# qlchan/cronsun

Hardware: AMD Instinct MI355X
Metric: fire events materialised/sec (1M rules × 24h) + HBM GB/s at 1/2/4/8 GPU (higher is better)
Workload: dtype int64

## Files before the change

### cronsun_amd/csrc/cg_api_internal.h

```cpp
#pragma once
#include <hip/hip_runtime.h>

#include <algorithm>
#include <mutex>
#include <string>
#include <vector>

#include "../../include/cronsun_gpu.h"
#include "cg_kernels.h"
#include "cg_zone.h"

int cg_fail(int code, const std::string& msg);
int cg_hip_check(hipError_t e, const char* what);

#define HIPCHK(x)                    \
  do {                               \
    int _rc = cg_hip_check((x), #x); \
    if (_rc != CG_OK) return _rc;    \
  } while (0)

struct alignas(16) RuleInfo {
  int32_t cnt, off, first, st;
};

struct alignas(16) PairRec {
  int32_t rule, dst, x, st;
};

inline int gridn(int64_t n, int threads, int cap) {
  int64_t b = (n + threads - 1) / threads;
  if (b < 1) b = 1;
  return int(std::min<int64_t>(b, cap));
}

template <class T>
struct DBuf {
  T* p = nullptr;
  size_t cap = 0;
  int ensure(size_t n) {
    if (n <= cap) return CG_OK;
    if (p) (void)hipFree(p);
    p = nullptr;
    size_t want = std::max(n, cap + cap / 4);
    hipError_t e = hipMalloc(&p, want * sizeof(T));
    if (e != hipSuccess) {
      e = hipMalloc(&p, n * sizeof(T));
      if (e != hipSuccess) {
        p = nullptr;
        cap = 0;
        return cg_hip_check(e, "hipMalloc");
      }
      want = n;
    }
    cap = want;
    return CG_OK;
  }
  void release() {
    if (p) (void)hipFree(p);
    p = nullptr;
    cap = 0;
  }
};

struct RulesStore {
  DBuf<int64_t> nid_off, gid_off, ex_off, group_off;
  DBuf<int32_t> nids, gids, ex, group_nodes, rule_job;
  DBuf<int32_t> next_same, prev_same;
  bool has_dup = false;
  DBuf<uint8_t> group_exists, job_pause;
  int32_t n_nodes = 0, n_groups = 0, n_rules = 0, n_jobs = 0;
  uint64_t serial = 0;
  void release() {
    nid_off.release(); gid_off.release(); ex_off.release(); group_off.release();
    nids.release(); gids.release(); ex.release(); group_nodes.release(); rule_job.release();
    next_same.release(); prev_same.release();
    group_exists.release(); job_pause.release();
  }
};

struct RunSet {
  DBuf<int64_t> run_anchor, run_off, offsets, block_run;
  DBuf<int32_t> run_count;
  DBuf<uint32_t> run_dmask;
  DBuf<char> scan_tmp, plan_dev;
  DBuf<unsigned long long> stuck;
  int64_t* res_host = nullptr;
  int64_t* res_dev = nullptr;
  char* plan_pin = nullptr;
  size_t plan_pin_cap = 0;
  cg::Plan plan;
  cg::PlanArgs pa{};
  bool plan_valid = false;
  uint64_t plan_zone = 0;
  int64_t plan_t0 = 0, plan_t1 = 0;
  bool plan_lock_table = false;
  bool armed = false;
  int64_t R = 0, cap = 0;
  bool has_walk() const { return (plan.flags & (cg::kPlanT0Walk | cg::kPlanWalkSegs)) != 0; }
  int ensure_res() {
    if (res_host) return CG_OK;
    HIPCHK(hipHostMalloc(reinterpret_cast<void**>(&res_host), 16, hipHostMallocMapped | hipHostMallocCoherent));
    HIPCHK(hipHostGetDevicePointer(reinterpret_cast<void**>(&res_dev), res_host, 0));
    res_host[0] = 0;
    res_host[1] = -1;
    return CG_OK;
  }
  void release() {
    run_anchor.release(); run_off.release(); offsets.release(); block_run.release();
    run_count.release(); run_dmask.release(); scan_tmp.release(); plan_dev.release(); stuck.release();
    if (res_host) (void)hipHostFree(res_host);
    if (plan_pin) (void)hipHostFree(plan_pin);
    res_host = res_dev = nullptr;
    plan_pin = nullptr;
    plan_pin_cap = 0;
  }
};

struct AsyncSet {
  RunSet rs;
  hipEvent_t written = nullptr;
  hipEvent_t done = nullptr;
  int tslot = 0;
  int tprev = -1;
  bool pending = false;
  void release() {
    rs.release();
    if (written) (void)hipEventDestroy(written), written = nullptr;
    done = nullptr;
  }
};

struct PnWindow {
  DBuf<RuleInfo> rule_info;
  DBuf<int64_t> seg_cnt, seg_pos;
  DBuf<int32_t> seg_nrec;
  DBuf<PairRec> recs;
  DBuf<uint32_t> tickets;
  int64_t* node_off = nullptr;
  void* scan_tmp = nullptr;
  int64_t* res_host = nullptr;
  int64_t* res_dev = nullptr;
  const int64_t* offsets = nullptr;
  const int64_t* times = nullptr;
  int64_t t0 = 0;
  int32_t N = 0, K = 0, B = 0;
  int ensure_res() {
    if (res_host) return CG_OK;
    HIPCHK(hipHostMalloc(reinterpret_cast<void**>(&res_host), 32, hipHostMallocMapped | hipHostMallocCoherent));
    HIPCHK(hipHostGetDevicePointer(reinterpret_cast<void**>(&res_dev), res_host, 0));
    res_host[0] = res_host[1] = res_host[2] = 0;
    return CG_OK;
  }
  void release() {
    rule_info.release(); seg_cnt.release(); seg_pos.release(); seg_nrec.release();
    recs.release(); tickets.release();
    if (res_host) (void)hipHostFree(res_host);
    res_host = res_dev = nullptr;
  }
};

struct PnAsyncSet {
  RunSet rm;
  PnWindow w;
  DBuf<int64_t> times, node_off;
  DBuf<char> seg_tmp;
  hipEvent_t side_done = nullptr, written = nullptr, nw0 = nullptr, nw1 = nullptr;
  bool pending = false;
  bool timed = false;
  int64_t t0 = 0, t1 = 0, node_cap = 0, rm_cap = 0;
  int32_t N = 0;
  void release() {
    rm.release();
    w.release();
    times.release(); node_off.release(); seg_tmp.release();
    for (hipEvent_t* e : {&side_done, &written, &nw0, &nw1})
      if (*e) (void)hipEventDestroy(*e), *e = nullptr;
  }
};

struct cg_ctx {
  int device = 0;
  int write_blocks = 1024;
  int write_blocks_ov = 1024;
  hipStream_t st = nullptr;
  hipEvent_t ev[8] = {};
  hipEvent_t pev[4] = {};
  std::mutex mu;
  float kt[23] = {0, 0, 0, 0, 0, 0, 0, 0, 0, 0, 0, 0, 0, 0, 0, 0, 0, 0, 0, 0, 0, 0, 0};
  int phase_timing = 2;

  std::vector<char> plan_host;
  DBuf<char> plan_dev;

  RunSet rs;
  DBuf<int64_t> times, nb_in, nb_out, lt_avg;
  DBuf<int32_t> lt_kind;
  DBuf<char> scan_tmp;
  DBuf<unsigned long long> cksum;
  int64_t last_E = 0, last_R = 0;

#ifndef CG_ASYNC_SETS
#define CG_ASYNC_SETS 3
#endif
  static constexpr int kAsyncSets = CG_ASYNC_SETS;
  AsyncSet as[kAsyncSets];
  int as_next = 0, as_last = -1;
  hipStream_t st_cs = nullptr;
  hipEvent_t cs_done[kAsyncSets] = {};
  int async_rc = 0;
  std::string async_msg;
  double wr_ms_sum = 0;
  int wr_n = 0;
  hipStream_t st_w1 = nullptr;
  DBuf<int64_t> times2;
  bool ov_on = true;
  bool ov_active = false;
  bool w1_dirty = false;
  unsigned wr_call = 0;
  int times_last = 0;
  static constexpr int kTimeRing = kAsyncSets + 1;
  hipEvent_t tw0[kTimeRing] = {}, tw1[kTimeRing] = {};
  int tw_next = 0, tw_prev = -1;
  int64_t* result_times() const { return times_last ? times2.p : times.p; }

  static constexpr int kPnSets = 3;
  PnAsyncSet pns[kPnSets];
  int pa_next = 0, pa_last = -1;
  int pa_rc = 0;
  std::string pa_msg;
  double nw_ms_sum = 0;
  int nw_n = 0;
  int64_t pa_en_sum = 0;

  DBuf<int64_t> rn_off, node_off, node_time, nt_off, rs_off, seg_pair;
  DBuf<int32_t> rn_cnt, rn_nodes, pair_node, pair_rule, node_rule, nt_rule, rs_hist;
  PnWindow pn;
  DBuf<int32_t> ts_cnt, ts_tile_node, ts_hist, node_rule2;
  DBuf<int64_t> ts_base, ts_off, node_time2, ts_node_off;
  DBuf<int64_t> ts_start;
  DBuf<int32_t> ts_hi;
  int64_t pn_t0 = 0, pn_t1 = 0;
  RulesStore rules;
  int64_t pn_E = 0, pn_nnz = 0, pn_N = 0;
  bool pn_valid = false;
  int64_t pn_R = INT64_MAX;
  DBuf<int64_t> mr_rb, mr_tp, mr_t;
  DBuf<int32_t> mr_r;
  uint64_t pn_cache_serial = 0;
  int pn_cache_mode = -1;
  int node_order = CG_NODE_ORDER_RULE;
  bool pn_time_ordered = false;
  int32_t pn_B = 0, pn_K = 0;
  hipStream_t st_ot = nullptr;
  hipEvent_t ot_fork = nullptr, ot_join = nullptr;

  DBuf<int32_t> pf_rules, pf_chunk_cnt;
  DBuf<int64_t> pf_totals, pf_nodes, pf_part, pf_chunk_off;
  int64_t pf_R = 0;
  int32_t pf_N = 0, pf_B = 0;
  bool pf_valid = false, pf_has_nodes = false;
  int pf_kind = CG_PROFILE_STARTS;
  DBuf<int64_t> pf_dur, pf_peak;
  DBuf<int32_t> pf_peak_bucket;
  bool pf_peaks_valid = false;
  DBuf<char> pf_admit_units;
  DBuf<uint8_t> pf_admit_flag;
  DBuf<unsigned long long> pf_lock_stuck;
  hipEvent_t pfev[9] = {};
  uint64_t nt_gen = 0, pf_nt_gen = 0;
  int64_t pf_nnz = 0;
  DBuf<int32_t> tr_rule, tr_cnt, tr_nlisted, tr_ncontrib, tr_bucket, tr_part_nz;
  DBuf<unsigned long long> tr_part;
  int32_t tr_rows = 0, tr_k = 0;
  bool tr_valid = false;
  float tr_ms[3] = {0, 0, 0};
  hipEvent_t trev[3] = {};

  void free_all() {
    tr_rule.release(); tr_cnt.release(); tr_nlisted.release(); tr_ncontrib.release();
    tr_bucket.release(); tr_part_nz.release(); tr_part.release();
    for (hipEvent_t& e : trev)
      if (e) (void)hipEventDestroy(e), e = nullptr;
    for (AsyncSet& a : as) a.release();
    for (PnAsyncSet& a : pns) a.release();
    for (hipEvent_t& e : cs_done)
      if (e) (void)hipEventDestroy(e), e = nullptr;
    for (hipEvent_t* ring : {tw0, tw1})
      for (int i = 0; i < kTimeRing; i++)
        if (ring[i]) (void)hipEventDestroy(ring[i]), ring[i] = nullptr;
    if (st_cs) (void)hipStreamDestroy(st_cs);
    st_cs = nullptr;
    if (st_w1) (void)hipStreamDestroy(st_w1);
    st_w1 = nullptr;
    times2.release();
    if (ot_fork) (void)hipEventDestroy(ot_fork), ot_fork = nullptr;
    if (ot_join) (void)hipEventDestroy(ot_join), ot_join = nullptr;
    if (st_ot) (void)hipStreamDestroy(st_ot);
    st_ot = nullptr;
    plan_dev.release();
    rs.release(); times.release();
    nb_in.release(); nb_out.release(); lt_avg.release(); lt_kind.release();
    scan_tmp.release(); cksum.release();
    rn_off.release(); node_off.release(); node_time.release(); nt_off.release(); rs_off.release();
    seg_pair.release(); rn_cnt.release(); rn_nodes.release();
    pair_node.release(); pair_rule.release(); node_rule.release(); nt_rule.release();
    rs_hist.release(); pn.release(); rules.release();
    ts_cnt.release(); ts_tile_node.release(); ts_hist.release(); node_rule2.release();
    ts_start.release(); ts_hi.release();
    ts_base.release(); ts_off.release(); node_time2.release(); ts_node_off.release();
    mr_rb.release(); mr_tp.release(); mr_t.release(); mr_r.release();
    pf_rules.release(); pf_chunk_cnt.release(); pf_totals.release(); pf_nodes.release();
    pf_part.release(); pf_chunk_off.release();
    pf_dur.release(); pf_peak.release(); pf_peak_bucket.release();
    pf_admit_units.release(); pf_admit_flag.release(); pf_lock_stuck.release();
    for (hipEvent_t& e : pfev)
      if (e) (void)hipEventDestroy(e), e = nullptr;
  }
};

struct cg_rules {
  cg_ctx* ctx = nullptr;
  RulesStore st;
};

struct cg_zone {
  cg::ZoneRules rules;
  uint64_t serial;
};

struct cg_specs {
  cg_ctx* ctx = nullptr;
  cg::DSpec* d = nullptr;
  size_t n = 0;
  bool owner = false;
};

int pack_spec(const cg_schedule& s, cg::DSpec* d);
int upload_plan(cg_ctx* c, const cg::Plan& plan, int64_t t0, int64_t t1, cg::PlanArgs* pa);
struct PlanLayout {
  size_t o_when, o_off, o_seg, o_dt, bytes;
};
PlanLayout plan_layout(const cg::Plan& plan);
void plan_pack(const cg::Plan& plan, const PlanLayout& L, char* dst);
int plan_args(const cg::Plan& plan, const PlanLayout& L, char* dev_base, int64_t t0, int64_t t1,
              cg::PlanArgs* pa);
int run_set_count_scan(RunSet& rs, const cg_specs* s, const cg_zone* z, int64_t t0, int64_t t1, int64_t map_cap,
                       hipStream_t st, hipEvent_t* ev, bool* empty, bool lock_table = false);
int sync_count_scan(cg_ctx* c, const cg_specs* s, const cg_zone* z, int64_t t0, int64_t t1, bool* empty,
                    int64_t map_cap = 0, bool lock_table = false);
void run_set_write_enqueue(const RunSet& rs, const cg_specs* s, int64_t cap, int64_t* out, int blocks,
                           hipStream_t st, hipEvent_t after_cf = nullptr);
std::string stuck_msg(unsigned long long rule);
int expand_device_locked(cg_ctx* c, const cg_specs* s, const cg_zone* z, int64_t t0, int64_t t1,
                         int64_t* n_events);
int async_drain(cg_ctx* c);
int ensure_async(cg_ctx* c);
bool async_pending(const cg_ctx* c);
int pn_async_drain(cg_ctx* c);
bool pn_async_pending(const cg_ctx* c);
int upload_rules(const cg_rules_in* in, RulesStore* st, hipStream_t s);
int rule_nodes_locked(cg_ctx* c, const RulesStore& st, int mode, int64_t* nnz_out);
int transpose_locked(cg_ctx* c, int64_t nnz, int32_t N);
constexpr int kNodeChunk = 512;
int profile_node_peaks_enqueue(cg_ctx* c);
int64_t radix_hist_words(int64_t n);
void radix_by_key_enqueue(hipStream_t st, uint32_t* k0, int32_t* v0, uint32_t* k1, int32_t* v1, int64_t n,
                          int32_t N, int32_t* hist, int64_t* off, void* scan_tmp, bool* in_second);
void launch_node_bounds(hipStream_t st, const uint32_t* keys, int64_t n, int32_t N, int64_t* off);
constexpr int kInTimes = 0, kIn16 = 1, kInPacked = 2;
bool pn_pack_ok(int64_t R);
struct TileCut {
  const int64_t* seg_pos = nullptr;
  int32_t K = 1, B = 1;
  int64_t R = 0;
};
int order_merge_enqueue(cg_ctx* c, const int64_t* node_off, int32_t N, int64_t cap, int64_t t0, int64_t H,
                        hipStream_t st, int in_mode, int64_t* err, const TileCut& cut = TileCut());
constexpr const char* kOrderCheckMsg =
    "time-order pass: a sorted chunk came out of (time, rule) order (its LDS-atomic ranks were not in lane order)";
int order_by_time_locked(cg_ctx* c, int in_mode = 0);
int launch_node_place(cg_ctx* c, hipStream_t st, int32_t N, const int64_t* src_off, int64_t src_shift,
                      const int64_t* src_time, const int32_t* src_rule, int32_t rule_add, const int64_t* dst_start,
                      int64_t* dst_time, int32_t* dst_rule);
int launch_span_place(cg_ctx* c, hipStream_t st, int64_t n, const int64_t* src_time, const int32_t* src_rule,
                      int32_t rule_add, int64_t* dst_time, int32_t* dst_rule);
int launch_node_counts(cg_ctx* c, hipStream_t st, int64_t* d_counts);
int merge_ranks_locked(cg_ctx* c, hipStream_t st, int32_t N, int32_t W, const int64_t* h_rb, int64_t* d_time,
                       int32_t* d_rule, int64_t scratch_ev, DBuf<int64_t>& scr_t, DBuf<int32_t>& scr_r);
constexpr int kMergeMaxRanks = 64;
bool order_lsd_only();
```

### cronsun_amd/csrc/cg_pernode.hip

```cpp
#include <hip/hip_runtime.h>

#include <algorithm>
#include <atomic>
#include <cstdlib>
#include <cstring>
#include <unordered_map>
#include <vector>

#include "../../include/cronsun_gpu.h"
#include "cg_api_internal.h"
#include "cg_kernels.h"

using namespace cg;

namespace {


__global__ void k_seg_bounds(const int64_t* __restrict__ nt_off, const int32_t* __restrict__ nt_rule,
                             int32_t N, int32_t K, int32_t B, int64_t* __restrict__ seg_pair) {
  const int64_t t = blockIdx.x * int64_t(blockDim.x) + threadIdx.x;
  const int64_t NK = int64_t(N) * K;
  if (t > NK) return;
  if (t == NK) {
    seg_pair[t] = nt_off[N];
    return;
  }
  const int32_t n = int32_t(t / K), k = int32_t(t - int64_t(n) * K);
  int64_t lo = nt_off[n], hi = nt_off[n + 1];
  const int64_t x = int64_t(k) * B;
  while (lo < hi) {
    const int64_t mid = (lo + hi) >> 1;
    if (int64_t(nt_rule[mid]) < x) lo = mid + 1;
    else hi = mid;
  }
  seg_pair[t] = lo;
}

#ifndef CG_NODE_AP
#define CG_NODE_AP 1
#endif
constexpr int kApRules = 256;
inline int64_t rule_info_slots(int64_t R) { return std::max<int64_t>(R, 1); }
__global__ __launch_bounds__(256) void k_rule_info(const int64_t* __restrict__ rule_off,
                                                    const int64_t* __restrict__ times, int64_t R, int64_t t0,
                                                    int32_t B, int64_t cap, RuleInfo* __restrict__ info,
                                                    int64_t* __restrict__ err) {
  __shared__ int64_t off[kApRules + 1];
  __shared__ int64_t step[kApRules];
  __shared__ int32_t ok[kApRules];
  const int64_t r0 = int64_t(blockIdx.x) * kApRules;
  const int nr = int(R - r0 < kApRules ? R - r0 : kApRules);
  const int tid = threadIdx.x;
  if (rule_off[R] > cap) {
    if (tid < nr) info[r0 + tid] = RuleInfo{0, 0, 0, 0};
    return;
  }
  const int64_t band_lo = rule_off[(r0 / B) * B];
  if (r0 % B == 0 && threadIdx.x == 0 && rule_off[r0 + B < R ? r0 + B : R] - band_lo > (int64_t(1) << 30))
    err[0] = 1;
  int64_t first = 0, cnt = 0;
  if (tid < nr) {
    const int64_t a = rule_off[r0 + tid];
    cnt = rule_off[r0 + tid + 1] - a;
    first = cnt > 0 ? times[a] : 0;
    off[tid] = a;
    step[tid] = cnt > 1 ? times[a + 1] - first : 1;
    ok[tid] = CG_NODE_AP;
  }
  if (tid == 0) off[nr] = rule_off[r0 + nr];
  __syncthreads();
  const int64_t e_end = off[nr];
  constexpr int kRiUnroll = 4;
  for (int64_t e0 = off[0] + tid; e0 + 1 < e_end; e0 += int64_t(blockDim.x) * kRiUnroll) {
    int64_t ta[kRiUnroll], tb[kRiUnroll];
#pragma unroll
    for (int u = 0; u < kRiUnroll; u++) {
      const int64_t e = e0 + int64_t(u) * blockDim.x;
      const int64_t ec = e + 1 < e_end ? e : e_end - 2;
      ta[u] = times[ec];
      tb[u] = times[ec + 1];
    }
#pragma unroll
    for (int u = 0; u < kRiUnroll; u++) {
      const int64_t e = e0 + int64_t(u) * blockDim.x;
      if (e + 1 >= e_end) break;
      int lo = 0, hi = nr - 1;
      while (lo < hi) {
        const int mid = (lo + hi + 1) >> 1;
        if (off[mid] <= e) lo = mid;
        else hi = mid - 1;
      }
      if (e + 1 < off[lo + 1] && tb[u] - ta[u] != step[lo]) ok[lo] = 0;
    }
  }
  __syncthreads();
  if (tid < nr) {
    const int64_t rel = first - t0, s = step[tid];
    const bool prog = cnt > 0 && ok[tid] && rel >= 0 && rel <= INT32_MAX && s > 0 && s <= INT32_MAX;
    info[r0 + tid] = RuleInfo{int32_t(cnt), int32_t(off[tid] - band_lo),
                              prog ? int32_t(rel) : 0, prog ? int32_t(s) : 0};
  }
}

__device__ __forceinline__ int32_t scan_halves(int32_t x) {
  x += __builtin_amdgcn_update_dpp(0, x, 0x111, 0xf, 0xf, true);
  x += __builtin_amdgcn_update_dpp(0, x, 0x112, 0xf, 0xf, true);
  x += __builtin_amdgcn_update_dpp(0, x, 0x114, 0xf, 0xf, true);
  x += __builtin_amdgcn_update_dpp(0, x, 0x118, 0xf, 0xf, true);
  x += __builtin_amdgcn_update_dpp(0, x, 0x142, 0xa, 0xf, false);
  return x;
}
__device__ __forceinline__ int32_t half_total(int32_t incl) {
  const int32_t lo = __builtin_amdgcn_readlane(incl, 31), hi = __builtin_amdgcn_readlane(incl, 63);
  return (threadIdx.x & 63) < 32 ? lo : hi;
}

#ifndef CG_SEG_PAIRS_PER_LANE
#define CG_SEG_PAIRS_PER_LANE 8
#endif
constexpr int kSegPairsPerLane = CG_SEG_PAIRS_PER_LANE;
constexpr int kSegWavesPerSimd = 1;

__global__ __launch_bounds__(256, kSegWavesPerSimd) void k_seg_records(const int64_t* __restrict__ seg_pair,
                                                      const int32_t* __restrict__ nt_rule,
                                                      const int64_t* __restrict__ rule_off,
                                                      const RuleInfo* __restrict__ info, int32_t N,
                                                      int32_t K, int32_t B, int64_t R,
                                                      int64_t* __restrict__ seg_cnt,
                                                      int32_t* __restrict__ seg_nrec,
                                                      PairRec* __restrict__ recs,
                                                      uint32_t* __restrict__ tickets,
                                                      int64_t* __restrict__ err, int32_t xg) {
  if (blockIdx.x == 0)
    for (int i = threadIdx.x; i < kTicketGroups * kTicketStride; i += blockDim.x) tickets[i] = 0;
  const int32_t grp = int32_t(blockIdx.x % unsigned(xg));
  const int64_t nb_g = (int64_t(gridDim.x) - grp + xg - 1) / xg;
  const int64_t lb = blockIdx.x / unsigned(xg);
  const int64_t nbands = (int64_t(K) - grp + xg - 1) / xg;
  const int64_t NKg = nbands * N;
  constexpr int L = 32;
  constexpr int P = kSegPairsPerLane;
  const int lane = threadIdx.x & 63, hl = lane & (L - 1);
  const int64_t Hg = nb_g * (blockDim.x >> 6) * 2;
  const int64_t per = (NKg + Hg - 1) / Hg;
  const int64_t hid = (lb * int64_t(blockDim.x >> 6) + (threadIdx.x >> 6)) * 2 + (lane >> 5);
  const uint32_t below = (1u << hl) - 1u;
  struct Seg {
    int64_t s, p0, p1;
  };
  auto bounds = [&](int64_t u) -> Seg {
    const int64_t t = hid * per + u;
    Seg g{-1, 0, 0};
    if (u < per && t < NKg) {
      const int32_t i = int32_t(t / N), n = int32_t(t - int64_t(i) * N);
      const int32_t k = grp + xg * i;
      g.s = int64_t(n) * K + k;
      g.p0 = seg_pair[g.s];
      g.p1 = seg_pair[g.s + 1];
    }
    return g;
  };
  auto rules = [&](const Seg& g, int32_t pc, int32_t (&r)[P]) {
#pragma unroll
    for (int u = 0; u < P; u++) {
      const int64_t pp = g.p0 + pc + u * L + hl;
      r[u] = pp < g.p1 ? nt_rule[pp] : -1;
    }
  };
  Seg cur = bounds(0), nxt = bounds(1);
  int32_t r[P], rn[P];
  rules(cur, 0, r);
  for (int64_t u = 0; u < per; u++) {
    const Seg nn = bounds(u + 2);
    rules(nxt, 0, rn);
    int64_t run = 0;
    int32_t nrec = 0;
    const int32_t len = int32_t(cur.p1 - cur.p0);
    const int32_t rounds_len = max(__builtin_amdgcn_readlane(len, 0), __builtin_amdgcn_readlane(len, 32));
    for (int32_t pc = 0; pc < rounds_len; pc += L * P) {
      if (pc > 0) rules(cur, pc, r);
      RuleInfo g[P];
#pragma unroll
      for (int u = 0; u < P; u++)
        g[u] = r[u] >= 0 ? info[r[u]] : RuleInfo{0, 0, 0, 0};
#pragma unroll
      for (int u = 0; u < P; u++) {
        const int32_t incl = scan_halves(g[u].cnt);
        const int64_t d = run + (incl - g[u].cnt);
        const uint64_t ball = __ballot(g[u].cnt > 0);
        const uint32_t ne = uint32_t(lane < 32 ? ball : ball >> 32);
        if (g[u].cnt > 0) {
          const int64_t at = cur.p0 + nrec + __popc(ne & below);
          const int64_t x = int64_t(g[u].first) - d * g[u].st;
          const bool prog = g[u].st != 0 && x >= INT32_MIN && x <= INT32_MAX;
          recs[at] = PairRec{r[u], int32_t(d), int32_t(prog ? x : int64_t(g[u].off) - d), prog ? g[u].st : 0};
        }
        run += half_total(incl);
        nrec += __popc(ne);
      }
    }
    if (hl == 0 && cur.s >= 0) {
      seg_cnt[cur.s] = run;
      seg_nrec[cur.s] = nrec;
      if (run > (int64_t(1) << 30)) err[0] = 1;
    }
    cur = nxt;
    nxt = nn;
#pragma unroll
    for (int u = 0; u < P; u++) r[u] = rn[u];
  }
}

__global__ void k_node_off_from_seg(const int64_t* __restrict__ seg_pos, int32_t N, int32_t K,
                                    int64_t* __restrict__ node_off, int64_t* __restrict__ res) {
  const int64_t n = blockIdx.x * int64_t(blockDim.x) + threadIdx.x;
  if (n > N) return;
  node_off[n] = seg_pos[n * K];
  if (n == N) res[0] = seg_pos[n * K];
}

__device__ __forceinline__ int64_t rl64n(int64_t v, int i) {
  const uint32_t lo = uint32_t(__builtin_amdgcn_readlane(int(uint32_t(v)), i));
  const uint32_t hi = uint32_t(__builtin_amdgcn_readlane(int(uint32_t(uint64_t(v) >> 32)), i));
  return int64_t((uint64_t(hi) << 32) | lo);
}

template <int V, class T>
__device__ __forceinline__ void out_store(T* p, T v) {
  if (V & 2) {
    asm volatile("" ::"v"(v));
    return;
  }
  __builtin_nontemporal_store(v, p);
}
constexpr int kNodeMajorDefault = 1;
constexpr int kNodeMajorOrdered = 0;
constexpr int32_t kNodeBandMajorK = 128;
inline int node_major_for(int32_t K) { return K >= kNodeBandMajorK ? 0 : kNodeMajorDefault; }
constexpr int kNodeGroups = 8 < kTicketGroups ? 8 : kTicketGroups;

template <int V, class Put>
__device__ __forceinline__ void node_segment(int64_t p0, int32_t nrec, int32_t q_lo, int32_t q_hi,
                                             const int64_t* __restrict__ tb, const PairRec* __restrict__ recs,
                                             int64_t t0, uint32_t* marks, uint32_t& tag, uint64_t le, Put&& put) {
  const int lane = threadIdx.x & 63;
  int32_t pq = -1, prule = 0;
  int64_t ptime = 0;
  PairRec nx;
  int32_t nx_end = q_hi;
  auto fetch = [&](int32_t w) {
    nx = recs[p0 + (w + lane < nrec ? w + lane : nrec - 1)];
    nx_end = w + 64 < nrec ? recs[p0 + w + 64].dst + q_lo : q_hi;
  };
  fetch(0);
  for (int32_t w = 0; w < nrec; w += 64) {
    const int32_t rr = nx.rule, dst = nx.dst + q_lo, dlt = nx.x, sst = nx.st, we = nx_end;
    const int nc = nrec - w < 64 ? nrec - w : 64;
    const int32_t qw = __builtin_amdgcn_readlane(dst, 0);
    if (w + 64 < nrec) fetch(w + 64);
    const bool live = lane < nc;
    auto one = [&](int32_t b) {
      tag++;
      const bool mark = live && dst >= b && dst < b + 64;
      marks[mark ? dst - b : 64 + lane] = tag;
      __builtin_amdgcn_fence(__ATOMIC_RELEASE, "wavefront");
      __builtin_amdgcn_wave_barrier();
      __builtin_amdgcn_fence(__ATOMIC_ACQUIRE, "wavefront");
      const int32_t q = b + lane;
      const uint64_t M = __ballot(marks[lane] == tag);
      const int before = __popcll(__ballot(live && dst < b));
      int own = before - 1 + __popcll(M & le);
      own = own < 0 ? 0 : (own >= nc ? nc - 1 : own);
      const int32_t dl = __builtin_amdgcn_ds_bpermute(own << 2, dlt);
      const int32_t sv = __builtin_amdgcn_ds_bpermute(own << 2, sst);
      int32_t rv = __builtin_amdgcn_ds_bpermute(own << 2, rr);
      const bool in = q >= qw && q < we;
      int64_t val = in && sv != 0 ? t0 + int64_t(dl) + int64_t(q - q_lo) * sv : 0;
      const int32_t gi = in && sv == 0 ? q + dl - q_lo : -1;
      if (__ballot(gi >= 0)) {
        if (gi >= 0) val = (V & 1) ? int64_t(gi) : tb[gi];
        asm volatile("" : "+v"(val));
      }
      if (b == pq) {
        val = q < qw ? ptime : val;
        rv = q < qw ? prule : rv;
      }
      if (b + 64 <= we || we == q_hi) {
        if ((b >= q_lo && b + 64 <= q_hi) || (q >= q_lo && q < q_hi)) {
          put(q, val, rv);
        }
        pq = -1;
      } else {
        pq = b;
        ptime = val;
        prule = rv;
      }
    };
    const int32_t b0 = qw & ~63, bl = we & ~63;
    if (qw & 63) one(b0);
    for (int32_t b = (qw + 63) & ~63; b < bl;) {
      const int o = __popcll(__ballot(live && dst <= b)) - 1;
      const int32_t e = o + 1 < nc ? __builtin_amdgcn_readlane(dst, o + 1) : we;
      if (e < b + 64) {
        one(b);
        b += 64;
        continue;
      }
      const int32_t bend = (e & ~63) < bl ? (e & ~63) : bl;
      const int32_t dl = __builtin_amdgcn_readlane(dlt, o), sv = __builtin_amdgcn_readlane(sst, o);
      const int32_t rv = __builtin_amdgcn_readlane(rr, o);
      if (sv != 0) {
        int64_t val = t0 + int64_t(dl) + int64_t(b + lane - q_lo) * sv;
        const int64_t step = int64_t(64) * sv;
        for (; b < bend; b += 64, val += step) {
          put(b + lane, val, rv);
        }
      } else {
        for (; b < bend; b += 64) {
          const int32_t gi = b + lane + dl - q_lo;
          int64_t val = (V & 1) ? int64_t(gi) : tb[gi];
          asm volatile("" : "+v"(val));
          put(b + lane, val, rv);
        }
      }
    }
    if ((we & 63) && (bl != b0 || !(qw & 63))) one(bl);
  }
}

template <int V, int OUT = kInTimes>
__global__ __launch_bounds__(256) void k_node_write(
    const int64_t* __restrict__ seg_pair, const int64_t* __restrict__ seg_pos,
    const int32_t* __restrict__ seg_nrec, const PairRec* __restrict__ recs, int64_t t0,
    const int64_t* __restrict__ rule_off, const int64_t* __restrict__ times, int32_t N, int32_t K,
    int32_t B, int64_t cap, uint32_t* __restrict__ tickets, int64_t* __restrict__ out_time,
    int32_t* __restrict__ out_rule, int node_major) {
  __shared__ uint32_t marks_all[4][128];
  const int lane = threadIdx.x & 63, wave = threadIdx.x >> 6;
  uint32_t* marks = marks_all[wave];
  marks[lane] = 0u;
  uint32_t tag = 0;
  const int64_t NK = int64_t(N) * K;
  if (seg_pos[NK] > cap) return;
  const uint64_t le = (2ull << lane) - 1ull;
  const int ng = int(gridDim.x) < kNodeGroups ? int(gridDim.x) : kNodeGroups;
  const int grp = int(gridDim.x >= 8u * unsigned(ng) ? (blockIdx.x >> 3) % unsigned(ng) : blockIdx.x % unsigned(ng));
  auto take = [&]() -> int64_t {
    unsigned int t = 0;
    if (lane == 0) t = atomicAdd(tickets + grp * kTicketStride, 1u);
    return grp + int64_t(ng) * int64_t(uint32_t(__builtin_amdgcn_readfirstlane(int(t))));
  };
  auto desc = [&](int64_t t) -> int64_t {
    if (t >= NK) return 0;
    const int32_t k = node_major ? int32_t(t % K) : int32_t(t / N);
    const int32_t n = node_major ? int32_t(t / K) : int32_t(t - int64_t(k) * N);
    const int64_t s = int64_t(n) * K + k;
    switch (lane) {
      case 0: return seg_pair[s];
      case 1: return seg_nrec[s];
      case 2: return seg_pos[s];
      case 3: return seg_pos[s + 1];
      case 4: return rule_off[int64_t(k) * B];
      default: return 0;
    }
  };
  int64_t t = take();
  int64_t dsc = desc(t);
  while (t < NK) {
    const int64_t t_next = take();
    const int64_t dsc_next = desc(t_next);
    const int64_t p0 = rl64n(dsc, 0), o0 = rl64n(dsc, 2), o1 = rl64n(dsc, 3), band_lo = rl64n(dsc, 4);
    const int32_t nrec = int32_t(rl64n(dsc, 1));
    t = t_next;
    dsc = dsc_next;
    if (o0 == o1) continue;
    const int64_t abase = o0 & ~int64_t(63);
    const int32_t q_lo = int32_t(o0 - abase), q_hi = q_lo + int32_t(o1 - o0);
    const int64_t* __restrict__ tb = times + band_lo;
    int64_t* __restrict__ ot = out_time + abase;
    uint16_t* __restrict__ o16 = reinterpret_cast<uint16_t*>(out_time) + abase;
    int32_t* __restrict__ orl = out_rule + abase;
    auto put = [&](int32_t q, int64_t val, int32_t rv) {
      if constexpr (OUT == kInPacked) {
        out_store<V>(orl + q, int32_t((uint32_t(val - t0 - 1) << 20) | (uint32_t(rv) & 0xFFFFFu)));
        return;
      }
      if constexpr (OUT == kIn16) out_store<V>(o16 + q, uint16_t(val - t0 - 1));
      else out_store<V>(ot + q, val);
      if (!(V & 8)) out_store<V>(orl + q, rv);
    };
    node_segment<V>(p0, nrec, q_lo, q_hi, tb, recs, t0, marks, tag, le, put);
  }
}

auto node_write_kernel(int out_mode, int variant) {
  if (out_mode == kInPacked) return &k_node_write<0, kInPacked>;
  if (out_mode == kIn16) return &k_node_write<0, kIn16>;
#ifdef CG_DIAG
  switch (variant) {
    case 1: return &k_node_write<1, kInTimes>;
    case 2: return &k_node_write<2, kInTimes>;
    case 3: return &k_node_write<3, kInTimes>;
    case 8: return &k_node_write<8, kInTimes>;
  }
#endif
  return &k_node_write<0, kInTimes>;
}

#ifndef CG_NODE_BPC
#define CG_NODE_BPC 0
#endif
int node_write_blocks_per_cu() {
  if (CG_NODE_BPC > 0) return CG_NODE_BPC + 2;
  int n = 0;
  if (hipOccupancyMaxActiveBlocksPerMultiprocessor(&n, node_write_kernel(kInTimes, 0), 256, 0) != hipSuccess || n < 1)
    n = 4;
  return std::min(n, 8);
}

#ifndef CG_BAND_MIN_RULES
#define CG_BAND_MIN_RULES 32768
#endif
#ifndef CG_BAND_BYTES
#define CG_BAND_BYTES (1536 * 1024)
#endif
__global__ void k_band_max(const int64_t* __restrict__ off, int64_t R, int32_t B, unsigned long long* out) {
  const int64_t k = blockIdx.x * int64_t(blockDim.x) + threadIdx.x;
  const int64_t a = k * B;
  if (a >= R) return;
  const int64_t b = a + B < R ? a + B : R;
  atomicMax(out, (unsigned long long)(off[b] - off[a]));
}

constexpr int32_t kSegXcdGroups = 8;
int32_t seg_xcd_groups(int32_t K) { return K >= 4 * kSegXcdGroups ? kSegXcdGroups : 1; }

int32_t band_rules(int64_t R, int64_t E) {
  const double per_rule = double(std::max<int64_t>(E, 1)) * 8.0 / double(std::max<int64_t>(R, 1));
  int64_t B = int64_t(double(CG_BAND_BYTES) / per_rule);
  int64_t p = CG_BAND_MIN_RULES;
  while (p < B && p < R && p < (int64_t(1) << 20)) p <<= 1;
  return int32_t(std::max<int64_t>(p, 1024));
}


int pn_records_enqueue(cg_ctx* c, PnWindow& w, const int64_t* offsets, const int64_t* times, int64_t cap, int64_t t0,
                       int64_t R, int32_t N, int32_t K, int32_t B, int64_t nnz, hipStream_t st, bool empty = false) {
  const int64_t NK = int64_t(N) * K;
  int rc;
  if ((rc = w.ensure_res()) || (rc = w.rule_info.ensure(rule_info_slots(R))) ||
      (rc = w.seg_cnt.ensure(std::max<int64_t>(NK, 1))) || (rc = w.seg_pos.ensure(NK + 1)) ||
      (rc = w.seg_nrec.ensure(std::max<int64_t>(NK, 1))) || (rc = w.recs.ensure(std::max<int64_t>(nnz, 1))) ||
      (rc = w.tickets.ensure(kTicketGroups * kTicketStride)))
    return rc;
  w.offsets = offsets, w.times = times, w.t0 = t0;
  w.N = N, w.K = K, w.B = B;
  w.res_host[0] = w.res_host[1] = w.res_host[2] = 0;
  if (empty) {
    HIPCHK(hipMemsetAsync(w.seg_pos.p, 0, (NK + 1) * 8, st));
    HIPCHK(hipMemsetAsync(w.rule_info.p, 0, rule_info_slots(R) * sizeof(RuleInfo), st));
    if (NK > 0) HIPCHK(hipMemsetAsync(w.seg_cnt.p, 0, NK * 8, st));
  } else {
    if (R > 0)
      hipLaunchKernelGGL(k_rule_info, dim3(unsigned((R + kApRules - 1) / kApRules)), dim3(256), 0, st, offsets, times,
                         R, t0, B, cap, w.rule_info.p, w.res_dev + 1);
    if (NK > 0)
      hipLaunchKernelGGL(k_seg_records, dim3(gridn(NK, 4, 256 * 64)), dim3(256), 0, st, c->seg_pair.p, c->nt_rule.p,
                         offsets, w.rule_info.p, N, K, B, R, w.seg_cnt.p, w.seg_nrec.p, w.recs.p, w.tickets.p,
                         w.res_dev + 1, seg_xcd_groups(K));
  }
  if (NK > 0 || !empty) launch_scan64(w.seg_cnt.p, w.seg_pos.p, NK, w.scan_tmp, st);
  hipLaunchKernelGGL(k_node_off_from_seg, dim3(gridn(int64_t(N) + 1, 256, 1 << 30)), dim3(256), 0, st, w.seg_pos.p,
                     N, K, w.node_off, w.res_dev);
  return CG_OK;
}

int node_write_variant() {
#ifdef CG_DIAG
  static const int variant = [] {
    const char* e = getenv("CG_NODE_VARIANT");
    return e ? atoi(e) : 0;
  }();
  return variant;
#else
  return 0;
#endif
}

void pn_writer_enqueue(cg_ctx* c, const PnWindow& w, int out_mode, int node_major, int per_cu, int64_t cap,
                       hipStream_t st) {
#ifdef CG_DIAG
  static const char* const env_per_cu = getenv("CG_NODE_BLOCKS_PER_CU");
  static const char* const env_order = getenv("CG_NODE_ORDER");
  if (env_per_cu) per_cu = std::max(1, atoi(env_per_cu));
  if (env_order && out_mode == kInTimes) node_major = atoi(env_order);
#endif
  const int64_t NK = int64_t(w.N) * w.K;
  const int nw_blocks = c->write_blocks / kWriteBlocksPerCU * per_cu;
  hipLaunchKernelGGL(node_write_kernel(out_mode, node_write_variant()),
                     dim3(unsigned(std::min<int64_t>(NK / 4 + 1, nw_blocks))), dim3(256), 0, st, c->seg_pair.p,
                     w.seg_pos.p, w.seg_nrec.p, w.recs.p, w.t0, w.offsets, w.times, w.N, w.K, w.B, cap, w.tickets.p,
                     c->node_time.p, c->node_rule.p, node_major);
}

std::string pn_size_error_msg(int32_t B) {
  return "per-node output: a (node, rule band) segment, or a band of " + std::to_string(B) +
         " consecutive rules, fires more than 2^30 times in this window (the writer's 32-bit band indices; "
         "narrow the time window)";
}

int per_node_locked(cg_ctx* c, const cg_specs* s, const cg_zone* z, int64_t t0, int64_t t1,
                    const RulesStore& in, int mode, int64_t* n_events, int64_t* nnz_out) {
  if (int64_t(s->n) != in.n_rules)
    return cg_fail(CG_EINVAL, "specs count != rules n_rules");
  int64_t E = 0;
  int rc = expand_device_locked(c, s, z, t0, t1, &E);
  if (rc) return rc;
  int64_t nnz = 0;
  const int32_t N = in.n_nodes;
  const int64_t R = in.n_rules;
  hipStream_t st = c->st;
  const bool cached = in.serial != 0 && in.serial == c->pn_cache_serial && mode == c->pn_cache_mode;
  c->pn_E = 0;
  c->pn_valid = false;
  c->pn_time_ordered = false;
  c->pn_R = R;
  (void)hipEventRecord(c->pev[0], st);
  if (cached) {
    nnz = c->pn_nnz;
  } else {
    c->pn_cache_serial = 0;
    c->pn_K = 0;
    if ((rc = rule_nodes_locked(c, in, mode, &nnz))) return rc;
  }
  (void)hipEventRecord(c->pev[1], st);
  if (!cached && (rc = transpose_locked(c, nnz, N))) return rc;
  int32_t B = band_rules(R, E);
  if (E > (int64_t(1) << 30) && R > 0) {
    if ((rc = c->cksum.ensure(1))) return rc;
    for (;;) {
      HIPCHK(hipMemsetAsync(c->cksum.p, 0, 8, st));
      hipLaunchKernelGGL(k_band_max, dim3(gridn((R + B - 1) / B, 256, 1 << 30)), dim3(256), 0, st,
                         c->rs.offsets.p, R, B, c->cksum.p);
      unsigned long long mx = 0;
      HIPCHK(hipMemcpyAsync(&mx, c->cksum.p, 8, hipMemcpyDeviceToHost, st));
      HIPCHK(hipStreamSynchronize(st));
      if (mx <= (1ull << 30) || B <= kApRules) break;
      B /= 2;
    }
  }
  const int32_t K = int32_t(std::max<int64_t>(1, (R + B - 1) / B));
  const int64_t NK = int64_t(N) * K;
  if ((rc = c->seg_pair.ensure(NK + 1)) || (rc = c->node_off.ensure(N + 1))) return rc;
  if ((rc = c->scan_tmp.ensure(std::max(c->scan_tmp.cap, scan_temp_bytes(NK))))) return rc;
  if (!(cached && c->pn_B == B && c->pn_K == K)) {
    hipLaunchKernelGGL(k_seg_bounds, dim3(gridn(NK + 1, 256, 1 << 30)), dim3(256), 0, st, c->nt_off.p,
                       c->nt_rule.p, N, K, B, c->seg_pair.p);
    c->pn_B = B;
    c->pn_K = K;
  }
  PnWindow& w = c->pn;
  w.node_off = c->node_off.p;
  w.scan_tmp = c->scan_tmp.p;
  if ((rc = pn_records_enqueue(c, w, c->rs.offsets.p, c->times.p, int64_t(c->times.cap), t0, R, N, K, B, nnz, st)))
    return rc;
  (void)hipEventRecord(c->pev[2], st);
  static const int per_cu = node_write_blocks_per_cu();
  const bool off16 =
      c->node_order == CG_NODE_ORDER_TIME && t1 - t0 <= 4096 && node_write_variant() == 0 && !order_lsd_only();
  const int in_mode = !off16 ? kInTimes : (pn_pack_ok(R) ? kInPacked : kIn16);
  const int node_major = off16 ? kNodeMajorOrdered : node_major_for(K);
  int64_t En = 0;
  for (int attempt = 0; attempt < 2; attempt++) {
    const int64_t cap = int64_t(std::min(c->node_time.cap, c->node_rule.cap));
    if (NK > 0 && cap > 0) pn_writer_enqueue(c, w, in_mode, node_major, per_cu, cap, st);
    (void)hipEventRecord(c->pev[3], st);
    if ((rc = cg_hip_check(hipGetLastError(), "per-node kernels"))) return rc;
    if ((rc = cg_hip_check(hipStreamSynchronize(st), "sync"))) return rc;
    En = w.res_host[0];
    if (w.res_host[1] != 0) return cg_fail(CG_ERANGE, pn_size_error_msg(B));
    if (En <= cap) break;
    if ((rc = c->node_time.ensure(En)) || (rc = c->node_rule.ensure(En))) return rc;
    HIPCHK(hipMemsetAsync(w.tickets.p, 0, kTicketGroups * kTicketStride * 4, st));
    (void)hipEventRecord(c->pev[2], st);
  }
  (void)hipEventElapsedTime(&c->kt[6], c->pev[0], c->pev[1]);
  (void)hipEventElapsedTime(&c->kt[7], c->pev[1], c->pev[2]);
  (void)hipEventElapsedTime(&c->kt[8], c->pev[2], c->pev[3]);
  c->pn_E = En;
  c->pn_valid = true;
  c->pn_nnz = nnz;
  c->pn_N = N;
  c->pn_t0 = t0;
  c->pn_t1 = t1;
  c->pn_cache_serial = in.serial;
  c->pn_cache_mode = mode;
  *n_events = En;
  *nnz_out = nnz;
  if (c->node_order == CG_NODE_ORDER_TIME) {
    if ((rc = order_by_time_locked(c, in_mode))) {
      c->pn_E = 0;
      c->pn_valid = false;
      *n_events = 0;
    }
    return rc;
  }
  c->kt[12] = 0.f;
  return CG_OK;
}

}


namespace {

void pn_check_set(cg_ctx* c, PnAsyncSet& a) {
  if (!a.pending) return;
  a.pending = false;
  float ms = 0.f;
  if (hipEventElapsedTime(&ms, a.nw0, a.nw1) == hipSuccess) {
    c->nw_ms_sum += ms;
    c->nw_n++;
  }
  const int64_t E = a.rm.res_host[0], En = a.w.res_host[0];
  c->pa_en_sum += En;
  if (c->pa_rc) return;
  const unsigned long long stuck = static_cast<unsigned long long>(a.rm.res_host[1]);
  if (stuck != ~0ULL) {
    c->pa_rc = CG_ERANGE;
    c->pa_msg = stuck_msg(stuck);
  } else if (E > a.rm_cap) {
    c->pa_rc = CG_ECAPACITY;
    c->pa_msg = "per-node async window (" + std::to_string(a.t0) + ", " + std::to_string(a.t1) + "]: " +
                std::to_string(E) + " rule-major events exceed the capacity " + std::to_string(a.rm_cap) +
                " (run a synchronous per-node call on a window this large first)";
  } else if (a.w.res_host[2] != 0) {
    c->pa_rc = CG_EHIP;
    c->pa_msg = kOrderCheckMsg;
  } else if (a.w.res_host[1] != 0) {
    c->pa_rc = CG_ERANGE;
    c->pa_msg = pn_size_error_msg(a.w.B);
  } else if (En > a.node_cap) {
    c->pa_rc = CG_ECAPACITY;
    c->pa_msg = "per-node async window (" + std::to_string(a.t0) + ", " + std::to_string(a.t1) + "]: " +
                std::to_string(En) + " node events exceed the output capacity " + std::to_string(a.node_cap) +
                " (run a synchronous per-node call on a window this large first)";
  }
}

int pn_ensure_async(cg_ctx* c) {
  int rc = ensure_async(c);
  if (rc) return rc;
  for (PnAsyncSet& a : c->pns) {
    if (a.written) continue;
    HIPCHK(hipEventCreateWithFlags(&a.side_done, hipEventDisableTiming));
    HIPCHK(hipEventCreateWithFlags(&a.written, hipEventDisableTiming));
    HIPCHK(hipEventCreateWithFlags(&a.nw0, hipEventDisableSystemFence));
    HIPCHK(hipEventCreateWithFlags(&a.nw1, hipEventDisableSystemFence));
  }
  return CG_OK;
}

}

bool pn_async_pending(const cg_ctx* c) {
  for (const PnAsyncSet& a : c->pns)
    if (a.pending) return true;
  return false;
}

int pn_async_drain(cg_ctx* c) {
  if (!pn_async_pending(c)) return CG_OK;
  HIPCHK(hipStreamSynchronize(c->st));
  for (PnAsyncSet& a : c->pns) pn_check_set(c, a);
  return CG_OK;
}

extern "C" {

int cg_expand_per_node_rules_device_async(cg_ctx* c, const cg_specs* s, const cg_zone* z, int64_t t0, int64_t t1,
                                          const cg_rules* rules, int mode) {
  if (!c || !s || !z || !rules) return cg_fail(CG_EINVAL, "cg_expand_per_node_rules_device_async: null");
  if (rules->ctx != c) return cg_fail(CG_EINVAL, "rule set uploaded on another context");
  std::lock_guard<std::mutex> g(c->mu);
  (void)hipGetLastError();
  HIPCHK(hipSetDevice(c->device));
  const RulesStore& in = rules->st;
  if (int64_t(s->n) != in.n_rules) return cg_fail(CG_EINVAL, "specs count != rules n_rules");
  if (!(in.serial != 0 && in.serial == c->pn_cache_serial && mode == c->pn_cache_mode && c->pn_K > 0))
    return cg_fail(CG_EINVAL, "cg_expand_per_node_rules_device_async: run cg_expand_per_node_rules_device once "
                              "on this rule set and exclude mode first (rule->node join, bands, capacity)");
  if (t1 - t0 > CG_MAX_HORIZON || t0 < -(int64_t(1) << 45) || t1 > (int64_t(1) << 45))
    return cg_fail(CG_ERANGE, "horizon must satisfy t1 - t0 <= CG_MAX_HORIZON (40 years)");
  if (async_pending(c))
    return cg_fail(CG_EINVAL, "pipelined rule-major calls pending (call cg_expand_wait first)");
  const int64_t rm_cap = int64_t(c->times.cap);
  const int64_t node_cap = int64_t(std::min(c->node_time.cap, c->node_rule.cap));
  if (rm_cap == 0 || node_cap == 0) return cg_fail(CG_ECAPACITY, "no output capacity yet (run a synchronous call)");
  int rc = pn_ensure_async(c);
  if (rc) return rc;
  c->as_last = -1;
  c->times_last = 0;
  c->last_R = 0;
  c->last_E = 0;
  const int k = c->pa_next;
  PnAsyncSet& a = c->pns[k];
  HIPCHK(hipEventSynchronize(a.written));
  pn_check_set(c, a);
  const int32_t N = in.n_nodes, K = c->pn_K, B = c->pn_B;
  const int64_t R = in.n_rules, NK = int64_t(N) * K, nnz = c->pn_nnz;
  hipStream_t sc = c->st_cs, st = c->st;
  const bool timed = c->node_order == CG_NODE_ORDER_TIME;
  c->pn_R = R;
  if (timed && t1 - t0 > 4096)
    return cg_fail(CG_EINVAL, "pipelined per-node windows in time order: windows of at most 4096 s");
  bool empty = false;
  if ((rc = run_set_count_scan(a.rm, s, z, t0, t1, rm_cap, sc, nullptr, &empty))) return rc;
  if ((rc = a.times.ensure(std::max<int64_t>(rm_cap, 1))) || (rc = a.node_off.ensure(int64_t(N) + 1)) ||
      (rc = a.seg_tmp.ensure(scan_temp_bytes(std::max<int64_t>(NK, 1)))))
    return rc;
  if (!empty) run_set_write_enqueue(a.rm, s, rm_cap, a.times.p, c->write_blocks, sc);
  PnWindow& w = a.w;
  w.node_off = a.node_off.p;
  w.scan_tmp = a.seg_tmp.p;
  if ((rc = pn_records_enqueue(c, w, a.rm.offsets.p, a.times.p, rm_cap, t0, R, N, K, B, nnz, sc, empty))) return rc;
  HIPCHK(hipEventRecord(a.side_done, sc));
  HIPCHK(hipStreamWaitEvent(st, a.side_done, 0));
  (void)hipEventRecord(a.nw0, st);
  if (NK > 0 && !empty) {
    static const int per_cu = std::max(1, node_write_blocks_per_cu() - 2);
    if (timed) {
      const int in_mode = pn_pack_ok(R) ? kInPacked : kIn16;
      pn_writer_enqueue(c, w, in_mode, kNodeMajorOrdered, per_cu, node_cap, st);
      if ((rc = order_merge_enqueue(c, a.node_off.p, N, node_cap, t0, t1 - t0, st, in_mode, w.res_dev + 2,
                                    TileCut{w.seg_pos.p, K, B, R})))
        return rc;
    } else {
      pn_writer_enqueue(c, w, kInTimes, node_major_for(K), per_cu, node_cap, st);
    }
  }
  (void)hipEventRecord(a.nw1, st);
  HIPCHK(hipEventRecord(a.written, st));
  HIPCHK(hipGetLastError());
  a.pending = true;
  a.timed = timed;
  a.t0 = t0;
  a.t1 = t1;
  a.rm_cap = rm_cap;
  a.node_cap = node_cap;
  a.N = N;
  c->pa_next = (k + 1) % cg_ctx::kPnSets;
  c->pa_last = k;
  c->pn_E = 0;
  c->pn_valid = false;
  return CG_OK;
}

int cg_expand_per_node_wait(cg_ctx* c, int64_t* n_events, int64_t* n_events_all) {
  if (!c) return cg_fail(CG_EINVAL, "cg_expand_per_node_wait: null");
  std::lock_guard<std::mutex> g(c->mu);
  (void)hipGetLastError();
  HIPCHK(hipSetDevice(c->device));
  int rc = pn_async_drain(c);
  if (rc) return rc;
  if (c->nw_n > 0) c->kt[8] = float(c->nw_ms_sum / c->nw_n);
  c->nw_ms_sum = 0;
  c->nw_n = 0;
  const int rc_async = c->pa_rc;
  const std::string msg = c->pa_msg;
  c->pa_rc = 0;
  c->pa_msg.clear();
// ... 140 lines not shown
```

Baseline: 866.1 billion.

## Skip non-firing rule lookups via LDS fire bitmap and full-wave segments

k_rule_info now also writes a per-rule bitmap of rules that fire in the window, built with a wave ballot. k_seg_records stages the bitmap slice for its bands in LDS and skips the RuleInfo gather for rules that do not fire. The kernel also moves from half-wave (32-lane) segments to full 64-lane segments, using a 6-step DPP scan and mbcnt for record positions. Pairs-per-lane and waves-per-SIMD launch bounds are retuned. The cost is an extra kernel output, LDS staging with a barrier, and different occupancy and register pressure.

```diff
diff --git a/cronsun_amd/csrc/cg_api_internal.h b/cronsun_amd/csrc/cg_api_internal.h
--- a/cronsun_amd/csrc/cg_api_internal.h
+++ b/cronsun_amd/csrc/cg_api_internal.h
@@ -132,6 +132,7 @@
 
 struct PnWindow {
   DBuf<RuleInfo> rule_info;
+  DBuf<uint64_t> fire_mask;
   DBuf<int64_t> seg_cnt, seg_pos;
   DBuf<int32_t> seg_nrec;
   DBuf<PairRec> recs;
@@ -152,7 +153,7 @@
     return CG_OK;
   }
   void release() {
-    rule_info.release(); seg_cnt.release(); seg_pos.release(); seg_nrec.release();
+    rule_info.release(); fire_mask.release(); seg_cnt.release(); seg_pos.release(); seg_nrec.release();
     recs.release(); tickets.release();
     if (res_host) (void)hipHostFree(res_host);
     res_host = res_dev = nullptr;
diff --git a/cronsun_amd/csrc/cg_pernode.hip b/cronsun_amd/csrc/cg_pernode.hip
--- a/cronsun_amd/csrc/cg_pernode.hip
+++ b/cronsun_amd/csrc/cg_pernode.hip
@@ -41,9 +41,11 @@
 #endif
 constexpr int kApRules = 256;
 inline int64_t rule_info_slots(int64_t R) { return std::max<int64_t>(R, 1); }
+inline int64_t fire_mask_words(int64_t R) { return std::max<int64_t>((R + kApRules - 1) / kApRules, 1) * (kApRules / 64); }
 __global__ __launch_bounds__(256) void k_rule_info(const int64_t* __restrict__ rule_off,
                                                     const int64_t* __restrict__ times, int64_t R, int64_t t0,
                                                     int32_t B, int64_t cap, RuleInfo* __restrict__ info,
+                                                    uint64_t* __restrict__ fire_mask,
                                                     int64_t* __restrict__ err) {
   __shared__ int64_t off[kApRules + 1];
   __shared__ int64_t step[kApRules];
@@ -53,6 +55,7 @@
   const int tid = threadIdx.x;
   if (rule_off[R] > cap) {
     if (tid < nr) info[r0 + tid] = RuleInfo{0, 0, 0, 0};
+    if ((tid & 63) == 0) fire_mask[(r0 + tid) >> 6] = 0;
     return;
   }
   const int64_t band_lo = rule_off[(r0 / B) * B];
@@ -100,31 +103,38 @@
     info[r0 + tid] = RuleInfo{int32_t(cnt), int32_t(off[tid] - band_lo),
                               prog ? int32_t(rel) : 0, prog ? int32_t(s) : 0};
   }
-}
-
-__device__ __forceinline__ int32_t scan_halves(int32_t x) {
+  const uint64_t fires = __ballot(tid < nr && int32_t(cnt) > 0);
+  if ((tid & 63) == 0) fire_mask[(r0 + tid) >> 6] = fires;
+}
+
+__device__ __forceinline__ int32_t scan_wave(int32_t x) {
   x += __builtin_amdgcn_update_dpp(0, x, 0x111, 0xf, 0xf, true);
   x += __builtin_amdgcn_update_dpp(0, x, 0x112, 0xf, 0xf, true);
   x += __builtin_amdgcn_update_dpp(0, x, 0x114, 0xf, 0xf, true);
   x += __builtin_amdgcn_update_dpp(0, x, 0x118, 0xf, 0xf, true);
   x += __builtin_amdgcn_update_dpp(0, x, 0x142, 0xa, 0xf, false);
+  x += __builtin_amdgcn_update_dpp(0, x, 0x143, 0xc, 0xf, false);
   return x;
 }
-__device__ __forceinline__ int32_t half_total(int32_t incl) {
-  const int32_t lo = __builtin_amdgcn_readlane(incl, 31), hi = __builtin_amdgcn_readlane(incl, 63);
-  return (threadIdx.x & 63) < 32 ? lo : hi;
-}
 
 #ifndef CG_SEG_PAIRS_PER_LANE
-#define CG_SEG_PAIRS_PER_LANE 8
+#define CG_SEG_PAIRS_PER_LANE 6
 #endif
 constexpr int kSegPairsPerLane = CG_SEG_PAIRS_PER_LANE;
-constexpr int kSegWavesPerSimd = 1;
+#ifndef CG_SEG_WAVES
+#define CG_SEG_WAVES 5
+#endif
+constexpr int kSegWavesPerSimd = CG_SEG_WAVES;
+#ifndef CG_SEG_MASK_WORDS
+#define CG_SEG_MASK_WORDS 2048
+#endif
+constexpr int kSegMaskWords = CG_SEG_MASK_WORDS;
 
 __global__ __launch_bounds__(256, kSegWavesPerSimd) void k_seg_records(const int64_t* __restrict__ seg_pair,
                                                       const int32_t* __restrict__ nt_rule,
                                                       const int64_t* __restrict__ rule_off,
-                                                      const RuleInfo* __restrict__ info, int32_t N,
+                                                      const RuleInfo* __restrict__ info,
+                                                      const uint64_t* __restrict__ fire_mask, int32_t N,
                                                       int32_t K, int32_t B, int64_t R,
                                                       int64_t* __restrict__ seg_cnt,
                                                       int32_t* __restrict__ seg_nrec,
@@ -138,34 +148,52 @@
   const int64_t lb = blockIdx.x / unsigned(xg);
   const int64_t nbands = (int64_t(K) - grp + xg - 1) / xg;
   const int64_t NKg = nbands * N;
-  constexpr int L = 32;
+  constexpr int L = 64;
   constexpr int P = kSegPairsPerLane;
-  const int lane = threadIdx.x & 63, hl = lane & (L - 1);
-  const int64_t Hg = nb_g * (blockDim.x >> 6) * 2;
+  const int lane = threadIdx.x & 63;
+  const int waves = blockDim.x >> 6;
+  const int64_t Hg = nb_g * waves;
   const int64_t per = (NKg + Hg - 1) / Hg;
-  const int64_t hid = (lb * int64_t(blockDim.x >> 6) + (threadIdx.x >> 6)) * 2 + (lane >> 5);
-  const uint32_t below = (1u << hl) - 1u;
+  const int64_t hid = lb * waves + __builtin_amdgcn_readfirstlane(threadIdx.x >> 6);
+  __shared__ uint64_t lmask[kSegMaskWords > 0 ? kSegMaskWords : 1];
+  const uint32_t* lmask32 = reinterpret_cast<const uint32_t*>(lmask);
+  const int32_t wpb = B >> 6;
+  const int64_t t_blk = lb * waves * per;
+  const int64_t t_blk_run = t_blk + waves * per;
+  const int64_t t_blk_end = t_blk_run < NKg ? t_blk_run : NKg;
+  const int32_t i_lo = t_blk < t_blk_end ? int32_t(t_blk / N) : 0;
+  const int64_t slots = t_blk < t_blk_end ? (t_blk_end - 1) / N - i_lo + 1 : 0;
+  const bool masked = kSegMaskWords > 0 && slots * wpb <= kSegMaskWords;
+  if (masked) {
+    const int64_t nwords = ((R + kApRules - 1) / kApRules) * (kApRules / 64);
+    const int32_t nw = int32_t(slots) * wpb;
+    for (int32_t j = threadIdx.x; j < nw; j += blockDim.x) {
+      const int32_t slot = j / wpb;
+      const int64_t gw = int64_t(grp + xg * (i_lo + slot)) * wpb + (j - slot * wpb);
+      lmask[j] = gw < nwords ? fire_mask[gw] : 0;
+    }
+    __syncthreads();
+  }
   struct Seg {
-    int64_t s, p0, p1;
+    int32_t i;
+    int64_t p0, p1;
   };
   auto bounds = [&](int64_t u) -> Seg {
     const int64_t t = hid * per + u;
     Seg g{-1, 0, 0};
     if (u < per && t < NKg) {
-      const int32_t i = int32_t(t / N), n = int32_t(t - int64_t(i) * N);
-      const int32_t k = grp + xg * i;
-      g.s = int64_t(n) * K + k;
-      g.p0 = seg_pair[g.s];
-      g.p1 = seg_pair[g.s + 1];
+      g.i = int32_t(t / N);
+      const int64_t s = (t - int64_t(g.i) * N) * K + (grp + xg * g.i);
+      g.p0 = seg_pair[s];
+      g.p1 = seg_pair[s + 1];
     }
     return g;
   };
   auto rules = [&](const Seg& g, int32_t pc, int32_t (&r)[P]) {
+    const int32_t* __restrict__ base = nt_rule + g.p0 + pc;
+    const int32_t left = int32_t(g.p1 - g.p0) - pc;
 #pragma unroll
-    for (int u = 0; u < P; u++) {
-      const int64_t pp = g.p0 + pc + u * L + hl;
-      r[u] = pp < g.p1 ? nt_rule[pp] : -1;
-    }
+    for (int u = 0; u < P; u++) r[u] = u * L + lane < left ? base[u * L + lane] : -1;
   };
   Seg cur = bounds(0), nxt = bounds(1);
   int32_t r[P], rn[P];
@@ -176,32 +204,37 @@
     int64_t run = 0;
     int32_t nrec = 0;
     const int32_t len = int32_t(cur.p1 - cur.p0);
-    const int32_t rounds_len = max(__builtin_amdgcn_readlane(len, 0), __builtin_amdgcn_readlane(len, 32));
-    for (int32_t pc = 0; pc < rounds_len; pc += L * P) {
+    const int32_t mw = (cur.i - i_lo - (grp + xg * cur.i)) * (wpb * 2);
+    PairRec* __restrict__ seg_recs = recs + cur.p0;
+    for (int32_t pc = 0; pc < len; pc += L * P) {
       if (pc > 0) rules(cur, pc, r);
       RuleInfo g[P];
 #pragma unroll
-      for (int u = 0; u < P; u++)
-        g[u] = r[u] >= 0 ? info[r[u]] : RuleInfo{0, 0, 0, 0};
+      for (int u = 0; u < P; u++) {
+        bool fires = r[u] >= 0;
+        if (masked && fires) fires = (lmask32[mw + (r[u] >> 5)] >> (r[u] & 31)) & 1u;
+        g[u] = fires ? info[r[u]] : RuleInfo{0, 0, 0, 0};
+      }
 #pragma unroll
       for (int u = 0; u < P; u++) {
-        const int32_t incl = scan_halves(g[u].cnt);
+        const int32_t incl = scan_wave(g[u].cnt);
         const int64_t d = run + (incl - g[u].cnt);
-        const uint64_t ball = __ballot(g[u].cnt > 0);
-        const uint32_t ne = uint32_t(lane < 32 ? ball : ball >> 32);
+        const uint64_t ne = __ballot(g[u].cnt > 0);
         if (g[u].cnt > 0) {
-          const int64_t at = cur.p0 + nrec + __popc(ne & below);
+          const int32_t at = nrec + int32_t(__builtin_amdgcn_mbcnt_hi(uint32_t(ne >> 32),
+                                                                      __builtin_amdgcn_mbcnt_lo(uint32_t(ne), 0)));
           const int64_t x = int64_t(g[u].first) - d * g[u].st;
           const bool prog = g[u].st != 0 && x >= INT32_MIN && x <= INT32_MAX;
-          recs[at] = PairRec{r[u], int32_t(d), int32_t(prog ? x : int64_t(g[u].off) - d), prog ? g[u].st : 0};
+          seg_recs[at] = PairRec{r[u], int32_t(d), int32_t(prog ? x : int64_t(g[u].off) - d), prog ? g[u].st : 0};
         }
-        run += half_total(incl);
-        nrec += __popc(ne);
+        run += __builtin_amdgcn_readlane(incl, 63);
+        nrec += __popcll(ne);
       }
     }
-    if (hl == 0 && cur.s >= 0) {
-      seg_cnt[cur.s] = run;
-      seg_nrec[cur.s] = nrec;
+    if (lane == 0 && cur.i >= 0) {
+      const int64_t s = (hid * per + u - int64_t(cur.i) * N) * K + (grp + xg * cur.i);
+      seg_cnt[s] = run;
+      seg_nrec[s] = nrec;
       if (run > (int64_t(1) << 30)) err[0] = 1;
     }
     cur = nxt;
@@ -449,6 +482,7 @@
   const int64_t NK = int64_t(N) * K;
   int rc;
   if ((rc = w.ensure_res()) || (rc = w.rule_info.ensure(rule_info_slots(R))) ||
+      (rc = w.fire_mask.ensure(fire_mask_words(R))) ||
       (rc = w.seg_cnt.ensure(std::max<int64_t>(NK, 1))) || (rc = w.seg_pos.ensure(NK + 1)) ||
       (rc = w.seg_nrec.ensure(std::max<int64_t>(NK, 1))) || (rc = w.recs.ensure(std::max<int64_t>(nnz, 1))) ||
       (rc = w.tickets.ensure(kTicketGroups * kTicketStride)))
@@ -459,14 +493,15 @@
   if (empty) {
     HIPCHK(hipMemsetAsync(w.seg_pos.p, 0, (NK + 1) * 8, st));
     HIPCHK(hipMemsetAsync(w.rule_info.p, 0, rule_info_slots(R) * sizeof(RuleInfo), st));
+    HIPCHK(hipMemsetAsync(w.fire_mask.p, 0, fire_mask_words(R) * 8, st));
     if (NK > 0) HIPCHK(hipMemsetAsync(w.seg_cnt.p, 0, NK * 8, st));
   } else {
     if (R > 0)
       hipLaunchKernelGGL(k_rule_info, dim3(unsigned((R + kApRules - 1) / kApRules)), dim3(256), 0, st, offsets, times,
-                         R, t0, B, cap, w.rule_info.p, w.res_dev + 1);
+                         R, t0, B, cap, w.rule_info.p, w.fire_mask.p, w.res_dev + 1);
     if (NK > 0)
       hipLaunchKernelGGL(k_seg_records, dim3(gridn(NK, 4, 256 * 64)), dim3(256), 0, st, c->seg_pair.p, c->nt_rule.p,
-                         offsets, w.rule_info.p, N, K, B, R, w.seg_cnt.p, w.seg_nrec.p, w.recs.p, w.tickets.p,
+                         offsets, w.rule_info.p, w.fire_mask.p, N, K, B, R, w.seg_cnt.p, w.seg_nrec.p, w.recs.p, w.tickets.p,
                          w.res_dev + 1, seg_xcd_groups(K));
   }
   if (NK > 0 || !empty) launch_scan64(w.seg_cnt.p, w.seg_pos.p, NK, w.scan_tmp, st);
```

Result: slower. 763.8 billion (-11.8%).
